# tungphambasement/DCNN

Measured on AMD Instinct MI355X. Metric: images/sec (whole node) ResNet-18 Tiny-ImageNet training at 1/2/4/8 MI355X, higher is better.
Workload: dtype bf16; 1 GPU; model=resnet18_tiny_imagenet, global_batch=256, per_gpu_batch=256, parallelism=dp1, optimizer=adam, hipgraph=True, engine=native (C++ host API)

## Files before the change

### dcnn_amd/csrc/host/dcnn/nn.hpp

```cpp
#pragma once
#include <functional>
#include <map>
#include <memory>
#include <string>
#include <vector>

#include "json.hpp"
#include "ops.hpp"
#include "tensor.hpp"

namespace dcnn {

struct ParamArena;
struct Param {
  std::string name;
  std::vector<int64_t> shape;
  Layout layout = Layout::NCHW;
  Tensor value, grad, shadow;
  Tensor m, v;
  std::shared_ptr<ParamArena> arena;
};

struct ParamArena {
  Tensor value, grad, m, v, shadow;
// ... 119 lines not shown
  std::string type() const override { return "grouped_conv2d"; }
  json::Value parameters_config() const override;
  bool backward_residual(const Tensor& dy, const Tensor& residual, Tensor& dx) override;
};

class Dense : public Layer {
 public:
  Dense(int in_features, int out_features, bool bias = true, std::string name = "dense");
  std::string type() const override { return "dense"; }
  json::Value parameters_config() const override;
  std::vector<int64_t> output_shape(const std::vector<int64_t>& in) const override;
  void build(const std::vector<int64_t>& in, Device dev, uint64_t seed) override;
  Tensor forward(const Tensor& x, bool training) override;
  Tensor backward(const Tensor& dy) override;
  double flops(const std::vector<int64_t>& in) const override { return 6.0 * in[0] * in_ * out_; }

 private:
  int in_, out_;
  bool bias_;
};

class BatchNorm : public Layer {
 public:
  explicit BatchNorm(int num_features, float eps = 1e-5f, float momentum = 0.1f, bool affine = true,
                     std::string name = "batchnorm");
  std::string type() const override { return "batchnorm"; }
  json::Value parameters_config() const override;
  std::vector<int64_t> output_shape(const std::vector<int64_t>& in) const override { return in; }
  double flops(const std::vector<int64_t>& in) const override {
    return 15.0 * (double)in[0] * (double)in[1] * (double)in[2] * (double)in[3];
  }
  void build(const std::vector<int64_t>& in, Device dev, uint64_t seed) override;
  Tensor forward(const Tensor& x, bool training) override;
  Tensor backward(const Tensor& dy) override;
// ... 89 lines not shown
};

class Pool2D : public Layer {
 public:
  Pool2D(bool max, int kh, int kw, int sh, int sw, int ph, int pw, std::string name);
  std::string type() const override { return max_ ? "maxpool2d" : "avgpool2d"; }
  json::Value parameters_config() const override;
  std::vector<int64_t> output_shape(const std::vector<int64_t>& in) const override;
  Tensor forward(const Tensor& x, bool training) override;
  Tensor backward(const Tensor& dy) override;
  bool is_max() const { return max_; }
  PoolShape shape_for(const std::vector<int64_t>& in) const;
  void set_fused_producer(class BatchNorm* bn) { bn_ = bn; }
  uint8_t* accept_prepooled(const Tensor& ypool, const std::vector<int64_t>& in);
  void clear_prepooled() { mbc().flag = false; }

 private:
  class BatchNorm* bn_ = nullptr;
  bool max_;
  int kh_, kw_, sh_, sw_, ph_, pw_;
};

class Flatten : public Layer {
 public:
  explicit Flatten(std::string name = "flatten") : Layer(std::move(name)) {}
  std::string type() const override { return "flatten"; }
  json::Value parameters_config() const override { return json::Value::object(); }
  std::vector<int64_t> output_shape(const std::vector<int64_t>& in) const override;
  Tensor forward(const Tensor& x, bool training) override;
  Tensor backward(const Tensor& dy) override;
};

class ResidualBlock : public Layer {
 public:
  ResidualBlock(std::vector<std::unique_ptr<Layer>> main, std::vector<std::unique_ptr<Layer>> shortcut,
                std::string activation = "relu", std::string name = "residual_block");
  std::string type() const override { return "residual_block"; }
  json::Value parameters_config() const override;
  std::vector<int64_t> output_shape(const std::vector<int64_t>& in) const override;
  double flops(const std::vector<int64_t>& in) const override;
  void build(const std::vector<int64_t>& in, Device dev, uint64_t seed) override;
  Tensor forward(const Tensor& x, bool training) override;
  Tensor backward(const Tensor& dy) override;
  void sync_shadow() override;
  void collect_params(std::vector<Param*>& out) override;
// ... 198 lines not shown
```

### dcnn_amd/csrc/host/dcnn/ops.hpp

```cpp
#pragma once
#include <cstdint>

namespace dcnn {

struct ConvShape {
  int N, C, H, W, Co, KH, KW, SH, SW, PH, PW, OH, OW;
};
struct PoolShape {
  int N, C, H, W, OH, OW, KH, KW, SH, SW, PH, PW;
};
enum ActKind { ACT_RELU = 0, ACT_LEAKY_RELU = 1, ACT_ELU = 2, ACT_SIGMOID = 3, ACT_TANH = 4, ACT_LINEAR = 5 };

namespace cpu_ops {
void conv_fwd(const float* x, const float* w, const float* b, float* y, const ConvShape& s);
void conv_bwd(const float* x, const float* w, const float* dy, float* dx, float* dw, float* db, const ConvShape& s);
void dwconv_fwd(const float* x, const float* w, const float* b, float* y, const ConvShape& s);
void dwconv_bwd(const float* x, const float* w, const float* dy, float* dx, float* dw, float* db, const ConvShape& s);
void gconv_fwd(const float* x, const float* w, const float* b, float* y, const ConvShape& s, int groups);
void gconv_bwd(const float* x, const float* w, const float* dy, float* dx, float* dw, float* db, const ConvShape& s,
               int groups);
void dense_fwd(const float* x, const float* w, const float* b, float* y, long N, long In, long Out);
void dense_bwd(const float* x, const float* w, const float* dy, float* dx, float* dw, float* db, long N, long In,
               long Out);
void bn_fwd(const float* x, float* y, long N, long C, long HW, const float* g, const float* b, float eps, bool train,
// ... 63 lines not shown
struct StemBn {
  const void* x;
  const float* mean;
  const float* istd;
  const float* gamma;
  float* dgamma;
  float* dbeta;
  const float* slab;
  int rows;
  bool train;
};
void stem_wgrad_bn(const void* dy, const float* x, float* gw, float* gb, const ConvShape& s, const StemBn& bn);
void dense_fwd(const void* x, const void* w, const float* bias, void* y, int N, int In, int Out);
void dense_dgrad(const void* dy, const void* w, void* dx, int N, int In, int Out);
void dense_wgrad(const void* dy, const void* x, float* gw, float* gb, int N, int In, int Out);
void bn_fwd(const void* x, void* y, long R, int C, const float* g, const float* b, float eps, bool train,
            float* rmean, float* rvar, float momentum, float* smean, float* sistd, bool relu = false,
            const void* residual = nullptr);
void bn_fwd_slab(const void* x, void* y, long R, int C, const float* slab, int rows, const float* g, const float* b,
                 float eps, float* rmean, float* rvar, float momentum, float* smean, float* sistd, bool relu,
                 const void* residual = nullptr);
void bn_bwd_slab(const void* dy, const void* x, void* dx, long R, int C, const float* mean, const float* istd,
                 const float* g, float* dg, float* db, bool train, const float* slab, int rows);
void bn_bwd(const void* dy, const void* x, void* dx, long R, int C, const float* mean, const float* istd,
            const float* g, float* dg, float* db, bool train, const void* yout = nullptr, void* dy_out = nullptr);
struct SecondaryStats {
  SecondaryStats();
  ~SecondaryStats();
};
struct BnRaw {
// ... 67 lines not shown
```

### dcnn_amd/csrc/host/nn.cpp

```cpp
#include "dcnn/nn.hpp"

#include "../kernels/fusion_plan.h"

#include <algorithm>
#include <chrono>
#include <cmath>
#include <cstdio>
#include <cstdlib>
#include <filesystem>
#include <fstream>
#include <iostream>
#include <sstream>
#include <stdexcept>

namespace dcnn {

namespace {
struct Rng {
  uint64_t s;
  explicit Rng(uint64_t seed) : s(seed * 0x9e3779b97f4a7c15ull + 0x632be59bd9b4e019ull) {}
  uint64_t next() {
    uint64_t z = (s += 0x9e3779b97f4a7c15ull);
    z = (z ^ (z >> 30)) * 0xbf58476d1ce4e5b9ull;
    z = (z ^ (z >> 27)) * 0x94d049bb133111ebull;
// ... 364 lines not shown
  if (in[1] * in[2] * in[3] != in_)
    throw std::runtime_error(name_ + ": " + std::to_string(in[1] * in[2] * in[3]) + " input features, expected " +
                             std::to_string(in_));
  return {in[0], out_, 1, 1};
}

void Dense::build(const std::vector<int64_t>& in, Device dev, uint64_t seed) {
  (void)in;
  dev_ = dev;
  params_.clear();
  const float bound = 1.f / std::sqrt((float)in_);
  add_param("weights", {out_, in_, 1, 1}, Layout::NCHW, uniform_init((size_t)out_ * in_, bound, seed));
  if (bias_) add_param("bias", {out_, 1, 1, 1}, Layout::NCHW, uniform_init((size_t)out_, bound, seed + 1));
}

Tensor Dense::forward(const Tensor& x, bool training) {
  (void)training;
  Tensor& x_ = mbc().a;
  check_act(x, dev_, "dense");
  const int N = (int)x.dim(0);
  output_shape(x.shape());
  Tensor y = act_empty({N, out_, 1, 1}, dev_);
  const float* b = bias_ ? params_[1].value.ptr<float>() : nullptr;
  if (dev_.is_gpu())
    gpu_ops::dense_fwd(x.data(), params_[0].shadow.data(), b, y.data(), N, in_, out_);
  else
    cpu_ops::dense_fwd(x.ptr<float>(), params_[0].value.ptr<float>(), b, y.ptr<float>(), N, in_, out_);
  x_ = x;
  return y;
}

Tensor Dense::backward(const Tensor& dy) {
  const Tensor& x_ = mbc().a;
  const int N = (int)x_.dim(0);
  float* gb = bias_ ? params_[1].grad.ptr<float>() : nullptr;
  if (dev_.is_gpu()) {
    gpu_ops::dense_wgrad(dy.data(), x_.data(), params_[0].grad.ptr<float>(), gb, N, in_, out_);
    if (!input_grad_) return Tensor();
    Tensor dx = act_empty(x_.shape(), dev_);
    gpu_ops::dense_dgrad(dy.data(), params_[0].shadow.data(), dx.data(), N, in_, out_);
    return dx;
  }
  Tensor dx = act_empty(x_.shape(), dev_);
  {
    cpu_ops::dense_bwd(x_.ptr<float>(), params_[0].value.ptr<float>(), dy.ptr<float>(), dx.ptr<float>(),
                       params_[0].grad.ptr<float>(), gb, N, in_, out_);
  }
  return dx;
}

// ... 274 lines not shown

json::Value Activation::parameters_config() const {
  json::Value p = json::Value::object();
  p["activation"] = kind_;
  return p;
}

static float act_alpha(int code) { return code == ACT_ELU ? 1.0f : 0.01f; }

bool Activation::is_relu() const { return code_ == ACT_RELU; }

static int fuse_kind(const Layer* l) {
  if (dynamic_cast<const Conv2D*>(l)) return FK_CONV;
  if (dynamic_cast<const BatchNorm*>(l)) return FK_BN;
  if (auto* a = dynamic_cast<const Activation*>(l)) return a->is_relu() ? FK_RELU : FK_ACT;
  if (auto* p = dynamic_cast<const Pool2D*>(l)) return p->is_max() ? FK_MAXPOOL : FK_OTHER;
  return FK_OTHER;
}

static std::vector<int> fuse_kinds(const std::vector<std::unique_ptr<Layer>>& seq) {
  std::vector<int> k;
  for (const auto& l : seq) k.push_back(fuse_kind(l.get()));
  return k;
}

void fuse_bn_relu(std::vector<std::unique_ptr<Layer>>& seq, bool on) {
  const std::vector<int> f = plan_sequence_fusions(fuse_kinds(seq));
  for (size_t i = 0; i < seq.size(); ++i) {
    Layer* l = seq[i].get();
    if (auto* conv = dynamic_cast<Conv2D*>(l)) {
      conv->set_stats_consumer(on && (f[i] & FF_EMIT_BN_STATS) ? static_cast<BatchNorm*>(seq[i + 1].get()) : nullptr);
      BatchNorm* prod = nullptr;
      if (on && (f[i] & FF_BNB_CONSUMER))
        prod = static_cast<BatchNorm*>(seq[fuse_kind(seq[i - 1].get()) == FK_BN ? i - 1 : i - 2].get());
      conv->set_bnb_producer(prod);
    } else if (auto* bn = dynamic_cast<BatchNorm*>(l)) {
      bn->set_fused_relu(on && (f[i] & FF_FUSE_RELU));
      Pool2D* pool = on && (f[i] & FF_FUSE_POOL) ? static_cast<Pool2D*>(seq[i + 2].get()) : nullptr;
      bn->set_fused_pool(pool);
      if (pool) pool->set_fused_producer(bn);
    } else if (auto* act = dynamic_cast<Activation*>(l)) {
      act->set_passthrough(on && (f[i] & FF_PASSTHROUGH));
    } else if (auto* pool = dynamic_cast<Pool2D*>(l)) {
      if (!on || i < 2 || !(f[i - 2] & FF_FUSE_POOL)) pool->set_fused_producer(nullptr);
    }
  }
}

Tensor Activation::forward(const Tensor& x, bool training) {
  (void)training;
  if (passthrough_ && dev_.is_gpu()) return x;
  Tensor& x_ = mbc().a;
  Tensor& y_ = mbc().b;
  check_act(x, dev_, "activation");
  Tensor y = act_empty(x.shape(), dev_);
  const long N = x.dim(0), C = x.dim(1), HW = x.dim(2) * x.dim(3);
  if (code_ == ACT_SOFTMAX) {
    if (dev_.is_gpu())
      gpu_ops::softmax_fwd(x.data(), y.data(), N * HW, (int)C);
// ... 390 lines not shown
  mc.b = ypool;
  mc.shape = in;
  mc.flag = true;
  return mc.a.ptr<uint8_t>();
}

Tensor Pool2D::forward(const Tensor& x, bool training) {
  (void)training;
  if (bn_ != nullptr && mbc().flag && mbc().b.defined() && mbc().b.data() == x.data())
    return x;
  mbc().flag = false;
  Tensor& idx_ = mbc().a;
  std::vector<int64_t>& in_shape_ = mbc().shape;
  check_act(x, dev_, "pool2d");
  const PoolShape p = shape_for(x.shape());
  Tensor y = act_empty({p.N, p.C, p.OH, p.OW}, dev_);
  in_shape_ = x.shape();
  if (max_) {
    const int64_t n = (int64_t)p.N * p.C * p.OH * p.OW;
    if (dev_.is_gpu()) {
      idx_.ensure({n}, DType::U8, dev_);
      gpu_ops::maxpool_fwd(x.data(), y.data(), idx_.ptr<uint8_t>(), p);
    } else {
      idx_.ensure({n}, DType::I32, dev_);
      cpu_ops::maxpool_fwd(x.ptr<float>(), y.ptr<float>(), idx_.ptr<int32_t>(), p);
    }
  } else if (dev_.is_gpu()) {
    gpu_ops::avgpool_fwd(x.data(), y.data(), p);
  } else {
    cpu_ops::avgpool_fwd(x.ptr<float>(), y.ptr<float>(), p);
  }
  return y;
}

Tensor Pool2D::backward(const Tensor& dy) {
  const Tensor& idx_ = mbc().a;
  const std::vector<int64_t>& in_shape_ = mbc().shape;
  const PoolShape p = shape_for(in_shape_);
  Tensor dx = act_empty(in_shape_, dev_);
  if (mbc().flag && bn_ != nullptr) {
    const gpu_ops::BnbOperands ops = bn_->bnb_operands(mb_);
    int rows = 0;
    const float* slab = gpu_ops::maxpool_bwd_bnb(dy.data(), idx_.ptr<uint8_t>(), mbc().b.data(), ops.x, ops.mean,
                                                 ops.istd, dx.data(), p, &rows);
    bn_->offer_bwd_stats(dx.data(), slab, rows);
    return dx;
  }
  if (max_) {
    if (dev_.is_gpu())
      gpu_ops::maxpool_bwd(dy.data(), idx_.ptr<uint8_t>(), dx.data(), p);
// ... 14 lines not shown
Tensor Flatten::forward(const Tensor& x, bool training) {
  (void)training;
  std::vector<int64_t>& in_shape_ = mbc().shape;
  check_act(x, dev_, "flatten");
  in_shape_ = x.shape();
  const auto os = output_shape(x.shape());
  const int64_t HW = x.dim(2) * x.dim(3);
  if (!dev_.is_gpu()) return x.view(os);
  if (HW == 1) return x.view(os, Layout::NHWC);
  Tensor y = act_empty(os, dev_);
  gpu_ops::nhwc_to_nchw(x.data(), y.data(), (int)x.dim(0), (int)HW, (int)x.dim(1));
  return y;
}

Tensor Flatten::backward(const Tensor& dy) {
  const std::vector<int64_t>& in_shape_ = mbc().shape;
  const int64_t HW = in_shape_[2] * in_shape_[3];
  if (!dev_.is_gpu()) return dy.view(in_shape_);
  if (HW == 1) return dy.view(in_shape_, Layout::NHWC);
  Tensor dx = act_empty(in_shape_, dev_);
  gpu_ops::nchw_to_nhwc_bf16(dy.data(), dx.data(), (int)in_shape_[0], (int)HW, (int)in_shape_[1]);
  return dx;
}

std::unique_ptr<Layer> create_layer(const json::Value& rec) {
  const std::string type = rec.get_string("type", "");
  const std::string name = rec.get_string("name", type);
  static const json::Value empty = json::Value::object();
  const json::Value& p = rec.has("parameters") ? rec.at("parameters") : empty;
  auto I = [&](const char* k, int64_t d) { return (int)p.get_int(k, d); };
// ... 711 lines not shown
```

### dcnn_amd/csrc/host/ops_gpu.hip

```cpp
#include <hip/hip_runtime.h>

#include <algorithm>
#include <cmath>
#include <cstdio>
#include <cstdlib>
#include <cstring>
#include <map>
#include <mutex>
#include <stdexcept>
#include <string>
#include <unordered_map>
#include <vector>

#include "../kernels/api.h"
#include "dcnn/ops.hpp"
#include "dcnn/tensor.hpp"

#define HOST_HIP_CHECK(x)                                                                    \
  do {                                                                                       \
    hipError_t e_ = (x);                                                                     \
    if (e_ != hipSuccess) throw std::runtime_error(std::string(#x) + ": " + hipGetErrorString(e_)); \
  } while (0)

namespace dcnn {
// ... 758 lines not shown
  conv_weight_transpose(kBF16, w, wt, Out, 1, In, cur());
  NtArgs a{static_cast<const bf16*>(dy), wt, dx, N, In, Out, Out, Out, In, kPlain, 0, 0, 0, 0, 1, 1, 1, 1, 1, 1, 0, 0,
           nullptr, nullptr, nullptr, 0, 0};
  gemm_nt(a, cur());
}

void dense_wgrad(const void* dy, const void* x, float* gw, float* gb, int N, int In, int Out) {
  const int splits = gemm_tn_splits(Out, In, N);
  wgrad_split(splits, (long)Out * In, Out, gw, gb, [&](float* slab, float* bslab) {
    TnArgs a{static_cast<const bf16*>(dy), static_cast<const bf16*>(x), slab, bslab, Out, In, N, kPlain, 0, 0, 0, 0,
             1, 1, 1, 1, 1, 1, 0, 0, In, 0};
    gemm_tn(a, splits, cur());
  });
}

static std::pair<const float*, int> reduce_stats(int mode, const float* slab, int rows, int C) {
  const int parts = bn_stat_parts(rows);
  float* sums = static_cast<float*>(scratch(STAT_SUMS, (size_t)2 * C * 4));
  float* part = parts > 1 ? static_cast<float*>(scratch(STAT_PART, (size_t)parts * 3 * C * 4)) : nullptr;
  bn_stat_reduce(mode, slab, rows, C, sums, part, nullptr, cur());
  return {parts > 1 ? part : sums, parts};
}

void bn_fwd(const void* x, void* y, long R, int C, const float* g, const float* b, float eps, bool train,
            float* rmean, float* rvar, float momentum, float* smean, float* sistd, bool relu, const void* residual) {
  if (!train) {
    bn_apply(kBF16, x, y, R, C, nullptr, 1, (float)R, g, b, eps, residual, relu ? 1 : 0, smean, sistd, rmean, rvar,
             momentum, 1, cur());
    return;
  }
// ... 228 lines not shown
```

### dcnn_amd/csrc/kernels/api.h

```cpp
#pragma once
#include <hip/hip_runtime.h>
#include <stdint.h>

#include "fusion_plan.h"
typedef __bf16 bf16;

namespace dcnn {
struct BnbArgs {
  const bf16* y; const bf16* x; const float* mean; const float* istd;
  const float* gamma; const float* beta; int mask_x;
};
struct NtArgs {
  const bf16* A; const bf16* B; void* C;
  int M, N, K; int lda, ldb, ldc; int mode;
  int nb, sh, sw, cs, gh, gw; int kh, kw, strh, strw, padh, padw;
  const float* bias; const bf16* residual; float* stats; int out_f32; int relu;
};
struct TnArgs {
  const bf16* dY; const bf16* X; float* slab; float* bias_slab;
  int M, N, P; int mode; int nb, sh, sw, cs, gh, gw; int kh, kw, strh, strw, padh, padw; int ldx; int k_per_split;
};
struct G2Args {
  const bf16* A; const bf16* B; bf16* C;
  unsigned a_bytes, b_bytes;
// ... 107 lines not shown
void transpose_batched(const float* in, float* out, int batch, int rows, int cols, hipStream_t s);
void transpose_batched16(const void* in, void* out, int batch, int rows, int cols, hipStream_t s);
void rows_copy(int kind, const void* src, int lds, void* dst, int ldd, long rows, int cols, hipStream_t s);
void nchw_cnhw(const float* in, float* out, int N, int C, int HW, int to_cnhw, hipStream_t s);
void pad_crop(const float* in, float* out, int NC, int H, int W, int OH, int OW, int top, int left, float value,
              hipStream_t s);
void gemm_g2f(const G2Args& a, hipStream_t s);
int gemm_g2f_stat_rows(int M, int N);
void gemm_t2f(T2Args a, int splits, hipStream_t s);
int gemm_t2f_splits(int M, int N, int P);
void set_f32_mode(int mode);
int get_f32_mode();
void conv_weight_transpose_f32(const float* w, float* wt, int Co, int T_, int Ci, hipStream_t s);
void gemm_tn(TnArgs a, int splits, hipStream_t s);
int gemm_tn_splits(int M, int N, int P);
struct ConvRouteGeom {
  int N, C, H, W, Co, KH, KW, SH, SW, PH, PW, OH, OW, g1s_mode;
};
enum ConvRoute : int { ROUTE_GENERIC = 0, ROUTE_GEMM_G2 = 1, ROUTE_HALO = 2, ROUTE_G1S = 3, ROUTE_HALO_S2 = 4 };
int conv_fwd_route(ConvRouteGeom g);
int conv_dgrad_route(ConvRouteGeom g);
int conv_wgrad_route(ConvRouteGeom g);
void splitk_reduce(const float* slab, float* out, long n, int splits, int accumulate, hipStream_t s);
void splitk_reduce2(const float* slab, float* out, long n, const float* bslab, float* bout, long nb, int splits,
                    int accumulate, hipStream_t s);

constexpr int kMaxRed = 48;
struct RedEnt { const float* slab; float* out; long n; int splits, unit0, chunks, groups, vec, wpc; };
struct MultiRed { int count; RedEnt e[kMaxRed]; };
void multi_splitk_reduce(MultiRed t, hipStream_t s);
// ... 28 lines not shown
                     const float* gamma, const float* beta, float eps, float* save_mean, float* save_istd,
                     float* run_mean, float* run_var, float momentum, hipStream_t s);
void gn_fwd(int dtype, const void* x, void* y, int N, int HW, int C, int G, const float* gamma, const float* beta,
            float eps, float* save_mean, float* save_istd, hipStream_t s);
void gn_bwd(int dtype, const void* dy, const void* x, void* dx, int N, int HW, int C, int G, const float* gamma,
            const float* mean, const float* istd, float* dgamma, float* dbeta, float* aff, hipStream_t s);

void maxpool_fwd(int dt, const void* x, void* y, uint8_t* idx, PoolGeom g, hipStream_t s);
void maxpool_bwd(int dt, const void* dy, const uint8_t* idx, void* dx, PoolGeom g, hipStream_t s);
bool maxpool_bwd_bnb_supported(PoolGeom g);
int maxpool_bwd_bnb_rows(PoolGeom g);
void maxpool_bwd_bnb(const bf16* dy, const uint8_t* idx, const bf16* ypool, const bf16* x, const float* mean,
                     const float* istd, bf16* dx, PoolGeom g, float* slab, float* zero_sums, hipStream_t s);
void avgpool_fwd(int dt, const void* x, void* y, PoolGeom g, hipStream_t s);
void avgpool_bwd(int dt, const void* dy, void* dx, PoolGeom g, hipStream_t s);
void act_fwd(int dt, const void* x, void* y, long n, int type, float a, hipStream_t s);
void act_bwd(int dt, const void* x, const void* dy, void* dx, long n, int type, float a, hipStream_t s);
void softmax_rows(int dt, const void* x, void* y, long rows, int C, hipStream_t s);
void softmax_rows_bwd(int dt, const void* y, const void* dy, void* dx, long rows, int C, hipStream_t s);
void dropout(int dt, const void* x, void* y, long n, float p, uint64_t seed, const uint64_t* ctr, hipStream_t s);
void counter_bump(uint64_t* ctr, uint64_t* slot, hipStream_t s);
void nchw_to_nhwc(int dt, const float* x, void* y, int N, int C, int HW, hipStream_t s);
void nchw_to_nhwc_pad(int dt, const float* x, void* y, int N, int C, int Cp, int HW, hipStream_t s);
void conv_weight_transpose(int src_dt, const void* w, bf16* wt, int Co, int T_, int Ci, hipStream_t s);
void cast_f32_bf16(const float* x, bf16* y, long n, hipStream_t s);
struct StemArgs {
  const float* x; const void* w; int w_bf16; long ws[4];
  const float* bias; bf16* y; float* slab; float* zero_ptr; int zero_n;
  const bf16* dy; float* bias_slab; long gs[4]; long n_slab;
  int halo_bytes; int N, Ci, H, W, Co, TH;
// ... 59 lines not shown
```

### dcnn_amd/csrc/kernels/bindings.cpp

```cpp
#include <tuple>
#include <pybind11/pybind11.h>
#include <pybind11/stl.h>
#include <algorithm>
#include <array>
#include <vector>
#include <hip/hip_runtime.h>
#include <stdint.h>

namespace py = pybind11;
#include "api.h"


using namespace dcnn;
void bind_runtime(py::module_& m);
void bind_rccl(py::module_& m);
template <typename T>
static inline T P(uintptr_t x) { return reinterpret_cast<T>(x); }
static inline hipStream_t S(uintptr_t x) { return reinterpret_cast<hipStream_t>(x); }

using Ptr4 = std::array<uintptr_t, 4>;
static BnbArgs bnb_of(const Ptr4& b) {
  return BnbArgs{P<const bf16*>(b[0]), P<const bf16*>(b[1]), P<const float*>(b[2]), P<const float*>(b[3])};
}

// ... 186 lines not shown
    std::vector<std::array<int, 6>> ph;
    for (const DgradPhase& c : p.phases) ph.push_back({c.ry, c.rx, c.GH, c.GW, c.t0, c.nt});
    return std::make_pair(ph, p.taps);
  });
  m.attr("ROUTE_GENERIC") = (int)ROUTE_GENERIC;
  m.attr("ROUTE_GEMM_G2") = (int)ROUTE_GEMM_G2;
  m.attr("ROUTE_HALO") = (int)ROUTE_HALO;
  m.attr("ROUTE_G1S") = (int)ROUTE_G1S;
  m.attr("ROUTE_HALO_S2") = (int)ROUTE_HALO_S2;
  m.def("plan_sequence_fusions", &plan_sequence_fusions);
  m.def("plan_residual_fusions", &plan_residual_fusions);
  for (auto [name, v] : {std::pair<const char*, int>{"FK_OTHER", FK_OTHER}, {"FK_CONV", FK_CONV}, {"FK_BN", FK_BN},
                         {"FK_RELU", FK_RELU}, {"FK_ACT", FK_ACT}, {"FK_MAXPOOL", FK_MAXPOOL},
                         {"FF_EMIT_BN_STATS", FF_EMIT_BN_STATS}, {"FF_FUSE_RELU", FF_FUSE_RELU},
                         {"FF_PASSTHROUGH", FF_PASSTHROUGH}, {"FF_FUSE_POOL", FF_FUSE_POOL},
                         {"FF_BNB_CONSUMER", FF_BNB_CONSUMER}, {"RF_FUSED_TAIL", RF_FUSED_TAIL},
                         {"RF_DUAL_SHORTCUT", RF_DUAL_SHORTCUT}})
    m.attr(name) = v;
  m.def("g1s_rows", &g1s_rows);
  m.def("g1s_enable", &g1s_enable);
  m.def("g1s_set_waves_per_simd", &g1s_set_waves_per_simd);
  m.def("g1s_gen_rows", &g1s_gen_rows);
  m.def("g1s_gen", [](uintptr_t X, uintptr_t Wt, uintptr_t Y, int NB, int GH, int GW, int N, int Kc, int ldw,
                      std::vector<std::array<int, 3>> taps, int H, int W, int OHo, int OWo, int OS, int ORY, int ORX,
                      uintptr_t residual, uintptr_t stats, uintptr_t zero_ptr, int zero_n, Ptr4 bnb,
                      int mode, uintptr_t stream) {
    g1s_gen(P<const bf16*>(X), P<const bf16*>(Wt), P<bf16*>(Y), NB, GH, GW, N, Kc, ldw, taps, H, W, OHo, OWo, OS, ORY,
            ORX, P<const bf16*>(residual), P<float*>(stats), P<float*>(zero_ptr), zero_n,
            bnb_of(bnb),
            mode, S(stream));
  });
// ... 182 lines not shown
  m.def("maxpool_bwd_bnb", [geom](uintptr_t dy, uintptr_t idx, uintptr_t ypool, uintptr_t x, uintptr_t mean,
                                  uintptr_t istd, uintptr_t dx, int N, int H, int W, int C, int OH, int OW, int ph,
                                  int pw, int sh, int sw, int padh, int padw, uintptr_t slab, uintptr_t zero_sums,
                                  uintptr_t st) {
    maxpool_bwd_bnb(P<const bf16*>(dy), P<const uint8_t*>(idx), P<const bf16*>(ypool), P<const bf16*>(x),
                    P<const float*>(mean), P<const float*>(istd), P<bf16*>(dx),
                    geom(N, H, W, C, OH, OW, ph, pw, sh, sw, padh, padw), P<float*>(slab), P<float*>(zero_sums), S(st));
  });
  m.def("avgpool_fwd", [geom](int dt, uintptr_t x, uintptr_t y, int N, int H, int W, int C, int OH, int OW, int ph,
                              int pw, int sh, int sw, int padh, int padw, uintptr_t st) {
    avgpool_fwd(dt, P<const void*>(x), P<void*>(y), geom(N, H, W, C, OH, OW, ph, pw, sh, sw, padh, padw), S(st));
  });
  m.def("avgpool_bwd", [geom](int dt, uintptr_t dy, uintptr_t dx, int N, int H, int W, int C, int OH, int OW, int ph,
                              int pw, int sh, int sw, int padh, int padw, uintptr_t st) {
    avgpool_bwd(dt, P<const void*>(dy), P<void*>(dx), geom(N, H, W, C, OH, OW, ph, pw, sh, sw, padh, padw), S(st));
  });
  m.def("act_fwd", [](int dt, uintptr_t x, uintptr_t y, long n, int type, float a, uintptr_t st) {
    act_fwd(dt, P<const void*>(x), P<void*>(y), n, type, a, S(st));
  });
  m.def("act_bwd", [](int dt, uintptr_t x, uintptr_t dy, uintptr_t dx, long n, int type, float a, uintptr_t st) {
    act_bwd(dt, P<const void*>(x), P<const void*>(dy), P<void*>(dx), n, type, a, S(st));
  });
  m.def("softmax_rows", [](int dt, uintptr_t x, uintptr_t y, long rows, int C, uintptr_t st) {
    softmax_rows(dt, P<const void*>(x), P<void*>(y), rows, C, S(st));
  });
  m.def("softmax_rows_bwd", [](int dt, uintptr_t y, uintptr_t dy, uintptr_t dx, long rows, int C, uintptr_t st) {
    softmax_rows_bwd(dt, P<const void*>(y), P<const void*>(dy), P<void*>(dx), rows, C, S(st));
  });
  m.def("dropout", [](int dt, uintptr_t x, uintptr_t y, long n, float p, uint64_t seed, uintptr_t ctr, uintptr_t st) {
    dropout(dt, P<const void*>(x), P<void*>(y), n, p, seed, P<const uint64_t*>(ctr), S(st));
// ... 128 lines not shown
```

### dcnn_amd/csrc/kernels/fusion_plan.cpp

```cpp
#include "fusion_plan.h"

namespace dcnn {

std::vector<int> plan_sequence_fusions(const std::vector<int>& kinds) {
  const size_t n = kinds.size();
  std::vector<int> f(n, 0);
  auto is = [&](size_t i, int k) { return i < n && kinds[i] == k; };
  for (size_t i = 0; i + 1 < n; ++i) {
    if (is(i, FK_CONV) && is(i + 1, FK_BN)) f[i] |= FF_EMIT_BN_STATS;
    if (is(i, FK_BN) && is(i + 1, FK_RELU)) {
      f[i] |= FF_FUSE_RELU;
      f[i + 1] |= FF_PASSTHROUGH;
    }
  }
  for (size_t i = 0; i + 2 < n; ++i)
    if (is(i, FK_BN) && is(i + 1, FK_RELU) && is(i + 2, FK_MAXPOOL)) f[i] |= FF_FUSE_POOL;
  for (size_t j = 1; j < n; ++j) {
    if (!is(j, FK_CONV)) continue;
    if (is(j - 1, FK_BN) || (j >= 2 && is(j - 1, FK_RELU) && is(j - 2, FK_BN))) f[j] |= FF_BNB_CONSUMER;
  }
  return f;
}

int plan_residual_fusions(const std::vector<int>& main_kinds, const std::vector<int>& short_kinds, bool act_ok) {
  const bool tail = act_ok && main_kinds.size() >= 2 && main_kinds.back() == FK_BN;
  if (!tail) return 0;
  const bool dual = !short_kinds.empty() && short_kinds.back() == FK_BN;
  return RF_FUSED_TAIL | (dual ? RF_DUAL_SHORTCUT : 0);
}

}
```

### dcnn_amd/csrc/kernels/fusion_plan.h

```cpp
#pragma once
#include <vector>

namespace dcnn {

enum FuseKind : int { FK_OTHER = 0, FK_CONV = 1, FK_BN = 2, FK_RELU = 3, FK_ACT = 4, FK_MAXPOOL = 5 };
enum FuseFlag : int {
  FF_EMIT_BN_STATS = 1,
  FF_FUSE_RELU = 2,
  FF_PASSTHROUGH = 4,
  FF_FUSE_POOL = 8,
  FF_BNB_CONSUMER = 16,
};
std::vector<int> plan_sequence_fusions(const std::vector<int>& kinds);
enum ResidualFlag : int { RF_FUSED_TAIL = 1, RF_DUAL_SHORTCUT = 2 };
int plan_residual_fusions(const std::vector<int>& main_kinds, const std::vector<int>& short_kinds, bool act_ok);

}
```

### dcnn_amd/csrc/kernels/gemm_conv.hip

```cpp
#include <algorithm>

#include "common.h"
#include "api.h"

namespace dcnn {

enum GatherMode { kPlain = 0, kConvFwd = 1, kConvDgrad = 2 };



__device__ __forceinline__ int xcd_remap(int bid, int nwg) {
  const int xcd = bid & 7, q = nwg >> 3, r = nwg & 7;
  const int base = xcd < r ? xcd * (q + 1) : r * (q + 1) + (xcd - r) * q;
  return base + (bid >> 3);
}

template <int BM, int BN, int BK, bool VEC>
struct NtTile {
  static constexpr int CPR = BK / 8;
  static constexpr int RPB = 256 / (BK * 2);
  static constexpr int A_CH = BM * CPR / 256;
  static constexpr int B_CH = BN * CPR / 256;
  static constexpr int TM = BM / 32, TN = BN / 32;
  static constexpr int LDS_BYTES = 2 * (BM + BN) * BK * 2;
// ... 625 lines not shown

int gemm_tn_splits(int M, int N, int P) {
  const int bm = M >= 128 ? 128 : 64, bn = N >= 128 ? 128 : 64;
  const long tiles = (long)((M + bm - 1) / bm) * ((N + bn - 1) / bn);
  long splits = (512 + tiles - 1) / tiles;
  const long min_k = tiles < 32 ? 64 : 64 * 4;
  const long max_by_k = P / min_k > 0 ? P / min_k : 1;
  if (splits > max_by_k) splits = max_by_k;
  const long max_by_mem = (64l << 20) / (4l * M * N) > 0 ? (64l << 20) / (4l * M * N) : 1;
  if (splits > max_by_mem) splits = max_by_mem;
  if (splits < 1) splits = 1;
  if (splits > 128) splits = 128;
  return (int)splits;
}

void gemm_tn(TnArgs a, int splits, hipStream_t s) {
  const bool conv = a.mode == kConvFwd;
  const int bm = a.M >= 128 ? 128 : 64;
  int bn = a.N >= 128 ? 128 : 64;
  if (conv) while (bn > 32 && a.cs % bn != 0) bn >>= 1;
  const bool v = a.M % 8 == 0 && (conv ? a.cs % bn == 0 : (a.N % 8 == 0 && a.ldx % 8 == 0));
  if (!v) bn = a.N >= 128 ? 128 : 64;
  const int per = (a.P + splits - 1) / splits;
  a.k_per_split = ((per + 63) / 64) * 64;
#define DCNN_TN(BM, BN, V) if (bm == BM && bn == BN && v == V) return launch_tn<BM, BN, 64, V>(a, splits, s)
  DCNN_TN(128, 128, true);
  DCNN_TN(128, 64, true);
  DCNN_TN(128, 32, true);
  DCNN_TN(64, 128, true);
  DCNN_TN(64, 64, true);
  DCNN_TN(64, 32, true);
  DCNN_TN(128, 128, false);
  DCNN_TN(128, 64, false);
  DCNN_TN(64, 128, false);
  DCNN_TN(64, 64, false);
#undef DCNN_TN
  throw std::runtime_error("gemm_tn: no kernel variant");
}

// ... 16 lines not shown
```

Before: 89810 images/sec.

## Fuse global avgpool, flatten and dense classifier head into single kernels

Adds a fused head path: the final whole-map average pool and the dense layer run in one forward kernel that writes both pooled features and logits. A single backward kernel computes the pool input gradient (dense dgrad broadcast over the spatial map) and the split weight gradients. Fusion planning tags an avgpool-flatten-dense tail, and the pool and flatten layers pass through when the fused path is active. This removes separate pool, dense GEMM and pool-backward launches and their intermediate traffic, at the cost of a specialised kernel with shape restrictions and extra cache bookkeeping between the layers.

```diff
diff --git a/dcnn_amd/csrc/host/dcnn/nn.hpp b/dcnn_amd/csrc/host/dcnn/nn.hpp
--- a/dcnn_amd/csrc/host/dcnn/nn.hpp
+++ b/dcnn_amd/csrc/host/dcnn/nn.hpp
@@ -157,10 +157,14 @@
   Tensor forward(const Tensor& x, bool training) override;
   Tensor backward(const Tensor& dy) override;
   double flops(const std::vector<int64_t>& in) const override { return 6.0 * in[0] * in_ * out_; }
+  void set_head_pool(class Pool2D* p) { head_pool_ = p; }
+  bool run_head(const Tensor& x, const PoolShape& p, Tensor& pooled);
+  bool is_head_dx(const Tensor& dy, bool take);
 
  private:
   int in_, out_;
   bool bias_;
+  class Pool2D* head_pool_ = nullptr;
 };
 
 class BatchNorm : public Layer {
@@ -280,9 +284,11 @@
   void set_fused_producer(class BatchNorm* bn) { bn_ = bn; }
   uint8_t* accept_prepooled(const Tensor& ypool, const std::vector<int64_t>& in);
   void clear_prepooled() { mbc().flag = false; }
+  void set_head_dense(class Dense* d) { head_ = d; }
 
  private:
   class BatchNorm* bn_ = nullptr;
+  class Dense* head_ = nullptr;
   bool max_;
   int kh_, kw_, sh_, sw_, ph_, pw_;
 };
@@ -295,6 +301,10 @@
   std::vector<int64_t> output_shape(const std::vector<int64_t>& in) const override;
   Tensor forward(const Tensor& x, bool training) override;
   Tensor backward(const Tensor& dy) override;
+  void set_head_dense(class Dense* d) { head_ = d; }
+
+ private:
+  class Dense* head_ = nullptr;
 };
 
 class ResidualBlock : public Layer {
diff --git a/dcnn_amd/csrc/host/dcnn/ops.hpp b/dcnn_amd/csrc/host/dcnn/ops.hpp
--- a/dcnn_amd/csrc/host/dcnn/ops.hpp
+++ b/dcnn_amd/csrc/host/dcnn/ops.hpp
@@ -101,6 +101,10 @@
 void dense_fwd(const void* x, const void* w, const float* bias, void* y, int N, int In, int Out);
 void dense_dgrad(const void* dy, const void* w, void* dx, int N, int In, int Out);
 void dense_wgrad(const void* dy, const void* x, float* gw, float* gb, int N, int In, int Out);
+bool head_supported(const PoolShape& p, int Out);
+void head_fwd(const void* x, const void* w, const float* bias, void* pooled, void* y, const PoolShape& p, int Out);
+void head_bwd(const void* dy, const void* w, const void* pooled, void* dx, float* gw, float* gb, const PoolShape& p,
+              int Out);
 void bn_fwd(const void* x, void* y, long R, int C, const float* g, const float* b, float eps, bool train,
             float* rmean, float* rvar, float momentum, float* smean, float* sistd, bool relu = false,
             const void* residual = nullptr);
diff --git a/dcnn_amd/csrc/host/nn.cpp b/dcnn_amd/csrc/host/nn.cpp
--- a/dcnn_amd/csrc/host/nn.cpp
+++ b/dcnn_amd/csrc/host/nn.cpp
@@ -402,8 +402,51 @@
   if (bias_) add_param("bias", {out_, 1, 1, 1}, Layout::NCHW, uniform_init((size_t)out_, bound, seed + 1));
 }
 
+static bool head_fuse_enabled() {
+  static const bool on = [] {
+    const char* v = std::getenv("DCNN_HEAD_FUSE");
+    return !(v && std::string(v) == "0");
+  }();
+  return on;
+}
+
+bool Dense::run_head(const Tensor& x, const PoolShape& p, Tensor& pooled) {
+  MbCache& mc = mbc();
+  mc.flag = false;
+  if (!dev_.is_gpu() || !head_fuse_enabled() || p.C != in_ || !gpu_ops::head_supported(p, out_)) return false;
+  pooled = act_empty({p.N, p.C, 1, 1}, dev_);
+  Tensor y = act_empty({p.N, out_, 1, 1}, dev_);
+  const float* b = bias_ ? params_[1].value.ptr<float>() : nullptr;
+  gpu_ops::head_fwd(x.data(), params_[0].shadow.data(), b, pooled.data(), y.data(), p, out_);
+  mc.a = pooled;
+  mc.b = y;
+  mc.shape = x.shape();
+  mc.flag = true;
+  return true;
+}
+
+bool Dense::is_head_dx(const Tensor& dy, bool take) {
+  MbCache& mc = mbc();
+  if (head_pool_ == nullptr || mc.u == 0) return false;
+  const bool same = mc.c.defined() ? dy.defined() && dy.data() == mc.c.data() : !dy.defined();
+  if (same && take) {
+    mc.c = Tensor();
+    mc.u = 0;
+  }
+  return same;
+}
+
 Tensor Dense::forward(const Tensor& x, bool training) {
   (void)training;
+  mbc().c = Tensor();
+  mbc().u = 0;
+  if (mbc().flag && mbc().b.defined() && x.data() == mbc().a.data()) {
+    Tensor y = mbc().b;
+    mbc().b = Tensor();
+    return y;
+  }
+  mbc().flag = false;
+  mbc().b = Tensor();
   Tensor& x_ = mbc().a;
   check_act(x, dev_, "dense");
   const int N = (int)x.dim(0);
@@ -422,6 +465,15 @@
   const Tensor& x_ = mbc().a;
   const int N = (int)x_.dim(0);
   float* gb = bias_ ? params_[1].grad.ptr<float>() : nullptr;
+  if (head_pool_ != nullptr && mbc().flag) {
+    const PoolShape p = head_pool_->shape_for(mbc().shape);
+    Tensor dx = input_grad_ ? act_empty(mbc().shape, dev_) : Tensor();
+    gpu_ops::head_bwd(dy.data(), params_[0].shadow.data(), x_.data(), input_grad_ ? dx.data() : nullptr,
+                      params_[0].grad.ptr<float>(), gb, p, out_);
+    mbc().c = dx;
+    mbc().u = 1;
+    return dx;
+  }
   if (dev_.is_gpu()) {
     gpu_ops::dense_wgrad(dy.data(), x_.data(), params_[0].grad.ptr<float>(), gb, N, in_, out_);
     if (!input_grad_) return Tensor();
@@ -726,7 +778,9 @@
   if (dynamic_cast<const Conv2D*>(l)) return FK_CONV;
   if (dynamic_cast<const BatchNorm*>(l)) return FK_BN;
   if (auto* a = dynamic_cast<const Activation*>(l)) return a->is_relu() ? FK_RELU : FK_ACT;
-  if (auto* p = dynamic_cast<const Pool2D*>(l)) return p->is_max() ? FK_MAXPOOL : FK_OTHER;
+  if (auto* p = dynamic_cast<const Pool2D*>(l)) return p->is_max() ? FK_MAXPOOL : FK_AVGPOOL;
+  if (dynamic_cast<const Flatten*>(l)) return FK_FLATTEN;
+  if (dynamic_cast<const Dense*>(l)) return FK_DENSE;
   return FK_OTHER;
 }
 
@@ -755,6 +809,11 @@
       act->set_passthrough(on && (f[i] & FF_PASSTHROUGH));
     } else if (auto* pool = dynamic_cast<Pool2D*>(l)) {
       if (!on || i < 2 || !(f[i - 2] & FF_FUSE_POOL)) pool->set_fused_producer(nullptr);
+      pool->set_head_dense(on && (f[i] & FF_FUSE_HEAD) ? static_cast<Dense*>(seq[i + 2].get()) : nullptr);
+    } else if (auto* flat = dynamic_cast<Flatten*>(l)) {
+      flat->set_head_dense(on && i >= 1 && (f[i - 1] & FF_FUSE_HEAD) ? static_cast<Dense*>(seq[i + 1].get()) : nullptr);
+    } else if (auto* dense = dynamic_cast<Dense*>(l)) {
+      dense->set_head_pool(on && i >= 2 && (f[i - 2] & FF_FUSE_HEAD) ? static_cast<Pool2D*>(seq[i - 2].get()) : nullptr);
     }
   }
 }
@@ -1175,8 +1234,13 @@
   std::vector<int64_t>& in_shape_ = mbc().shape;
   check_act(x, dev_, "pool2d");
   const PoolShape p = shape_for(x.shape());
+  in_shape_ = x.shape();
+  if (head_ != nullptr && training && !max_) {
+    head_->set_micro_batch(mb_);
+    Tensor pooled;
+    if (head_->run_head(x, p, pooled)) return pooled;
+  }
   Tensor y = act_empty({p.N, p.C, p.OH, p.OW}, dev_);
-  in_shape_ = x.shape();
   if (max_) {
     const int64_t n = (int64_t)p.N * p.C * p.OH * p.OW;
     if (dev_.is_gpu()) {
@@ -1195,6 +1259,10 @@
 }
 
 Tensor Pool2D::backward(const Tensor& dy) {
+  if (head_ != nullptr) {
+    head_->set_micro_batch(mb_);
+    if (head_->is_head_dx(dy, true)) return dy;
+  }
   const Tensor& idx_ = mbc().a;
   const std::vector<int64_t>& in_shape_ = mbc().shape;
   const PoolShape p = shape_for(in_shape_);
@@ -1239,6 +1307,10 @@
 }
 
 Tensor Flatten::backward(const Tensor& dy) {
+  if (head_ != nullptr) {
+    head_->set_micro_batch(mb_);
+    if (head_->is_head_dx(dy, false)) return dy;
+  }
   const std::vector<int64_t>& in_shape_ = mbc().shape;
   const int64_t HW = in_shape_[2] * in_shape_[3];
   if (!dev_.is_gpu()) return dy.view(in_shape_);
diff --git a/dcnn_amd/csrc/host/ops_gpu.hip b/dcnn_amd/csrc/host/ops_gpu.hip
--- a/dcnn_amd/csrc/host/ops_gpu.hip
+++ b/dcnn_amd/csrc/host/ops_gpu.hip
@@ -796,6 +796,21 @@
   });
 }
 
+bool head_supported(const PoolShape& p, int Out) { return dcnn::head_supported(geom(p), Out); }
+
+void head_fwd(const void* x, const void* w, const float* bias, void* pooled, void* y, const PoolShape& p, int Out) {
+  dcnn::head_fwd(static_cast<const bf16*>(x), static_cast<const bf16*>(w), bias, static_cast<bf16*>(pooled),
+                 static_cast<bf16*>(y), geom(p), Out, cur());
+}
+
+void head_bwd(const void* dy, const void* w, const void* pooled, void* dx, float* gw, float* gb, const PoolShape& p,
+              int Out) {
+  wgrad_split(head_bwd_splits(p.N, p.C, Out), (long)Out * p.C, Out, gw, gb, [&](float* slab, float* bslab) {
+    dcnn::head_bwd(static_cast<const bf16*>(dy), static_cast<const bf16*>(w), static_cast<const bf16*>(pooled),
+                   static_cast<bf16*>(dx), slab, bslab, geom(p), Out, cur());
+  });
+}
+
 static std::pair<const float*, int> reduce_stats(int mode, const float* slab, int rows, int C) {
   const int parts = bn_stat_parts(rows);
   float* sums = static_cast<float*>(scratch(STAT_SUMS, (size_t)2 * C * 4));
diff --git a/dcnn_amd/csrc/kernels/api.h b/dcnn_amd/csrc/kernels/api.h
--- a/dcnn_amd/csrc/kernels/api.h
+++ b/dcnn_amd/csrc/kernels/api.h
@@ -145,6 +145,8 @@
 void conv_weight_transpose_f32(const float* w, float* wt, int Co, int T_, int Ci, hipStream_t s);
 void gemm_tn(TnArgs a, int splits, hipStream_t s);
 int gemm_tn_splits(int M, int N, int P);
+int gemm_tn_k_per_split(int P, int splits);
+int gemm_tn_bias_rows(int M);
 struct ConvRouteGeom {
   int N, C, H, W, Co, KH, KW, SH, SW, PH, PW, OH, OW, g1s_mode;
 };
@@ -203,6 +205,12 @@
                      const float* istd, bf16* dx, PoolGeom g, float* slab, float* zero_sums, hipStream_t s);
 void avgpool_fwd(int dt, const void* x, void* y, PoolGeom g, hipStream_t s);
 void avgpool_bwd(int dt, const void* dy, void* dx, PoolGeom g, hipStream_t s);
+bool head_supported(PoolGeom g, int Out);
+void head_fwd(const bf16* x, const bf16* w, const float* bias, bf16* pooled, bf16* logits, PoolGeom g, int Out,
+              hipStream_t s);
+int head_bwd_splits(int N, int In, int Out);
+void head_bwd(const bf16* dlogits, const bf16* w, const bf16* pooled, bf16* dx, float* slab, float* bias_slab,
+              PoolGeom g, int Out, hipStream_t s);
 void act_fwd(int dt, const void* x, void* y, long n, int type, float a, hipStream_t s);
 void act_bwd(int dt, const void* x, const void* dy, void* dx, long n, int type, float a, hipStream_t s);
 void softmax_rows(int dt, const void* x, void* y, long rows, int C, hipStream_t s);
diff --git a/dcnn_amd/csrc/kernels/bindings.cpp b/dcnn_amd/csrc/kernels/bindings.cpp
--- a/dcnn_amd/csrc/kernels/bindings.cpp
+++ b/dcnn_amd/csrc/kernels/bindings.cpp
@@ -224,7 +224,9 @@
                          {"FK_RELU", FK_RELU}, {"FK_ACT", FK_ACT}, {"FK_MAXPOOL", FK_MAXPOOL},
                          {"FF_EMIT_BN_STATS", FF_EMIT_BN_STATS}, {"FF_FUSE_RELU", FF_FUSE_RELU},
                          {"FF_PASSTHROUGH", FF_PASSTHROUGH}, {"FF_FUSE_POOL", FF_FUSE_POOL},
-                         {"FF_BNB_CONSUMER", FF_BNB_CONSUMER}, {"RF_FUSED_TAIL", RF_FUSED_TAIL},
+                         {"FF_BNB_CONSUMER", FF_BNB_CONSUMER}, {"FK_AVGPOOL", FK_AVGPOOL},
+                         {"FK_FLATTEN", FK_FLATTEN}, {"FK_DENSE", FK_DENSE}, {"FF_FUSE_HEAD", FF_FUSE_HEAD},
+                         {"RF_FUSED_TAIL", RF_FUSED_TAIL},
                          {"RF_DUAL_SHORTCUT", RF_DUAL_SHORTCUT}})
     m.attr(name) = v;
   m.def("g1s_rows", &g1s_rows);
@@ -437,6 +439,23 @@
   m.def("avgpool_bwd", [geom](int dt, uintptr_t dy, uintptr_t dx, int N, int H, int W, int C, int OH, int OW, int ph,
                               int pw, int sh, int sw, int padh, int padw, uintptr_t st) {
     avgpool_bwd(dt, P<const void*>(dy), P<void*>(dx), geom(N, H, W, C, OH, OW, ph, pw, sh, sw, padh, padw), S(st));
+  });
+  m.def("head_supported", [geom](int N, int H, int W, int C, int OH, int OW, int ph, int pw, int sh, int sw, int padh,
+                                 int padw, int Out) {
+    return head_supported(geom(N, H, W, C, OH, OW, ph, pw, sh, sw, padh, padw), Out);
+  });
+  m.def("head_fwd", [geom](uintptr_t x, uintptr_t w, uintptr_t bias, uintptr_t pooled, uintptr_t logits, int N, int H,
+                           int W, int C, int OH, int OW, int ph, int pw, int sh, int sw, int padh, int padw, int Out,
+                           uintptr_t st) {
+    head_fwd(P<const bf16*>(x), P<const bf16*>(w), P<const float*>(bias), P<bf16*>(pooled), P<bf16*>(logits),
+             geom(N, H, W, C, OH, OW, ph, pw, sh, sw, padh, padw), Out, S(st));
+  });
+  m.def("head_bwd_splits", &head_bwd_splits);
+  m.def("head_bwd", [geom](uintptr_t dlogits, uintptr_t w, uintptr_t pooled, uintptr_t dx, uintptr_t slab,
+                           uintptr_t bias_slab, int N, int H, int W, int C, int OH, int OW, int ph, int pw, int sh,
+                           int sw, int padh, int padw, int Out, uintptr_t st) {
+    head_bwd(P<const bf16*>(dlogits), P<const bf16*>(w), P<const bf16*>(pooled), P<bf16*>(dx), P<float*>(slab),
+             P<float*>(bias_slab), geom(N, H, W, C, OH, OW, ph, pw, sh, sw, padh, padw), Out, S(st));
   });
   m.def("act_fwd", [](int dt, uintptr_t x, uintptr_t y, long n, int type, float a, uintptr_t st) {
     act_fwd(dt, P<const void*>(x), P<void*>(y), n, type, a, S(st));
diff --git a/dcnn_amd/csrc/kernels/fusion_plan.cpp b/dcnn_amd/csrc/kernels/fusion_plan.cpp
--- a/dcnn_amd/csrc/kernels/fusion_plan.cpp
+++ b/dcnn_amd/csrc/kernels/fusion_plan.cpp
@@ -19,6 +19,7 @@
     if (!is(j, FK_CONV)) continue;
     if (is(j - 1, FK_BN) || (j >= 2 && is(j - 1, FK_RELU) && is(j - 2, FK_BN))) f[j] |= FF_BNB_CONSUMER;
   }
+  if (n >= 3 && is(n - 3, FK_AVGPOOL) && is(n - 2, FK_FLATTEN) && is(n - 1, FK_DENSE)) f[n - 3] |= FF_FUSE_HEAD;
   return f;
 }
 
diff --git a/dcnn_amd/csrc/kernels/fusion_plan.h b/dcnn_amd/csrc/kernels/fusion_plan.h
--- a/dcnn_amd/csrc/kernels/fusion_plan.h
+++ b/dcnn_amd/csrc/kernels/fusion_plan.h
@@ -3,13 +3,17 @@
 
 namespace dcnn {
 
-enum FuseKind : int { FK_OTHER = 0, FK_CONV = 1, FK_BN = 2, FK_RELU = 3, FK_ACT = 4, FK_MAXPOOL = 5 };
+enum FuseKind : int {
+  FK_OTHER = 0, FK_CONV = 1, FK_BN = 2, FK_RELU = 3, FK_ACT = 4, FK_MAXPOOL = 5, FK_AVGPOOL = 6, FK_FLATTEN = 7,
+  FK_DENSE = 8
+};
 enum FuseFlag : int {
   FF_EMIT_BN_STATS = 1,
   FF_FUSE_RELU = 2,
   FF_PASSTHROUGH = 4,
   FF_FUSE_POOL = 8,
   FF_BNB_CONSUMER = 16,
+  FF_FUSE_HEAD = 32,
 };
 std::vector<int> plan_sequence_fusions(const std::vector<int>& kinds);
 enum ResidualFlag : int { RF_FUSED_TAIL = 1, RF_DUAL_SHORTCUT = 2 };
diff --git a/dcnn_amd/csrc/kernels/gemm_conv.hip b/dcnn_amd/csrc/kernels/gemm_conv.hip
--- a/dcnn_amd/csrc/kernels/gemm_conv.hip
+++ b/dcnn_amd/csrc/kernels/gemm_conv.hip
@@ -663,6 +663,9 @@
   return (int)splits;
 }
 
+int gemm_tn_k_per_split(int P, int splits) { return ((P + splits - 1) / splits + 63) / 64 * 64; }
+int gemm_tn_bias_rows(int M) { return 256 / (M >= 128 ? 128 : 64); }
+
 void gemm_tn(TnArgs a, int splits, hipStream_t s) {
   const bool conv = a.mode == kConvFwd;
   const int bm = a.M >= 128 ? 128 : 64;
@@ -670,8 +673,7 @@
   if (conv) while (bn > 32 && a.cs % bn != 0) bn >>= 1;
   const bool v = a.M % 8 == 0 && (conv ? a.cs % bn == 0 : (a.N % 8 == 0 && a.ldx % 8 == 0));
   if (!v) bn = a.N >= 128 ? 128 : 64;
-  const int per = (a.P + splits - 1) / splits;
-  a.k_per_split = ((per + 63) / 64) * 64;
+  a.k_per_split = gemm_tn_k_per_split(a.P, splits);
 #define DCNN_TN(BM, BN, V) if (bm == BM && bn == BN && v == V) return launch_tn<BM, BN, 64, V>(a, splits, s)
   DCNN_TN(128, 128, true);
   DCNN_TN(128, 64, true);
diff --git a/dcnn_amd/csrc/kernels/head.hip b/dcnn_amd/csrc/kernels/head.hip
--- /dev/null
+++ b/dcnn_amd/csrc/kernels/head.hip
@@ -0,0 +1,293 @@
+#include <algorithm>
+
+#include "api.h"
+#include "common.h"
+
+namespace dcnn {
+namespace {
+
+constexpr int kImgs = 16;
+constexpr int kFwdThreads = 512;
+constexpr int kFwdCls = 128;
+constexpr int kBwdThreads = 256;
+constexpr int kMaxIn = 2048;
+constexpr int kKC = 256;
+constexpr int kLdD = kKC + 8;
+constexpr int kLdW = 64 + 8;
+
+__device__ __forceinline__ f32x4 mfma16(bf16x8 a, bf16x8 b, f32x4 c) {
+  return __builtin_amdgcn_mfma_f32_16x16x32_bf16(a, b, c, 0, 0, 0);
+}
+__device__ __forceinline__ bf16x8 ld8(const bf16* p) { return *reinterpret_cast<const bf16x8*>(p); }
+
+__device__ __forceinline__ int swz(int r, int c) { return c ^ (r & 7); }
+
+__device__ __forceinline__ int wt_at(int i, int k) { return i * kLdD + (i >> 3) * 8 + k; }
+
+constexpr int kSmemData = (kImgs * kLdD + 64 * kLdD + 64 + kImgs * 64) * 2;
+constexpr int kSmemWeight = 2 * 64 * kLdW * 2;
+constexpr int kSmemBwd = kSmemData > kSmemWeight ? kSmemData : kSmemWeight;
+
+}
+
+__global__ __launch_bounds__(kFwdThreads) void head_fwd_kernel(const bf16* __restrict__ x, const bf16* __restrict__ w,
+                                                               const float* __restrict__ bias,
+                                                               bf16* __restrict__ pooled, bf16* __restrict__ logits,
+                                                               int N, int HW, int In, int Out, int ipb) {
+  extern __shared__ __attribute__((aligned(16))) unsigned char head_smem[];
+  bf16* tile = reinterpret_cast<bf16*>(head_smem);
+  const int n0 = blockIdx.x * ipb, nend = min(N, n0 + ipb);
+  const int chunks = In >> 3;
+  const int wave = threadIdx.x >> 6, lane = threadIdx.x & 63;
+  const int r = lane & 15, g = lane >> 4;
+  const int c0 = blockIdx.y * kFwdCls + wave * 16;
+  const bool wave_on = c0 < Out;
+  const int cls = c0 + r;
+  const bool cok = cls < Out;
+  const bf16* wr = w + (long)(cok ? cls : 0) * In + g * 8;
+  const int k64 = In >> 6;
+  bf16x8 b[16];
+  auto load_w = [&](int k0) {
+#pragma unroll
+    for (int u = 0; u < 8; ++u) {
+      const int kq = min(k0 + u, k64 - 1);
+      b[2 * u] = ld8(wr + kq * 64);
+      b[2 * u + 1] = ld8(wr + kq * 64 + 32);
+    }
+  };
+  if (wave_on) load_w(0);
+
+  for (int it = threadIdx.x; it < kImgs * chunks; it += kFwdThreads) {
+    const int pr = it / chunks, c = it - pr * chunks;
+    const int n = n0 + pr;
+    float s[8];
+#pragma unroll
+    for (int e = 0; e < 8; ++e) s[e] = 0.f;
+    if (n < nend) {
+      const uint4* px = reinterpret_cast<const uint4*>(x + (long)n * HW * In) + c;
+      for (int p0 = 0; p0 < HW; p0 += 8) {
+        uint4 u[8];
+#pragma unroll
+        for (int q = 0; q < 8; ++q) u[q] = p0 + q < HW ? px[(long)(p0 + q) * chunks] : make_uint4(0, 0, 0, 0);
+#pragma unroll
+        for (int q = 0; q < 8; ++q) {
+          float f[8];
+          unpack8(u[q], f);
+#pragma unroll
+          for (int e = 0; e < 8; ++e) s[e] += f[e];
+        }
+      }
+#pragma unroll
+      for (int e = 0; e < 8; ++e) s[e] = s[e] / (float)HW;
+    }
+    const uint4 o = pack8(s);
+    *reinterpret_cast<uint4*>(tile + pr * In + swz(pr, c) * 8) = o;
+    if (blockIdx.y == 0 && n < nend) *reinterpret_cast<uint4*>(pooled + (long)n * In + c * 8) = o;
+  }
+  __syncthreads();
+  if (!wave_on) return;
+
+  const bf16* ar = tile + r * In;
+  f32x4 acc = {0.f, 0.f, 0.f, 0.f};
+  for (int k0 = 0; k0 < k64; k0 += 8) {
+    if (k0 > 0) load_w(k0);
+#pragma unroll
+    for (int u = 0; u < 8; ++u) {
+      if (k0 + u < k64) {
+        acc = mfma16(ld8(ar + swz(r, (k0 + u) * 8 + g) * 8), b[2 * u], acc);
+        acc = mfma16(ld8(ar + swz(r, (k0 + u) * 8 + 4 + g) * 8), b[2 * u + 1], acc);
+      }
+    }
+  }
+  if (!cok) return;
+  const float bv = bias ? bias[cls] : 0.f;
+#pragma unroll
+  for (int j = 0; j < 4; ++j) {
+    const int n = n0 + g * 4 + j;
+    if (n < nend) logits[(long)n * Out + cls] = (bf16)(acc[j] + bv);
+  }
+}
+
+__global__ __launch_bounds__(kBwdThreads) void head_bwd_kernel(const bf16* __restrict__ dl, const bf16* __restrict__ w,
+                                                               const bf16* __restrict__ pooled, bf16* __restrict__ dx,
+                                                               float* __restrict__ slab, float* __restrict__ bslab,
+                                                               int N, int HW, int In, int Out, int n_data, int per,
+                                                               int brows) {
+  __shared__ __attribute__((aligned(16))) unsigned char smem[kSmemBwd];
+  const int tid = threadIdx.x, wave = tid >> 6, lane = tid & 63;
+  const int r = lane & 15, g = lane >> 4;
+  const int tiles_i = In >> 6;
+  const bf16 bz = (bf16)0.f;
+
+  if ((int)blockIdx.x < n_data) {
+    bf16* sdl = reinterpret_cast<bf16*>(smem);
+    bf16* swt = sdl + kImgs * kLdD;
+    bf16* sout = swt + 64 * kLdD + 64;
+    const int ib = blockIdx.x / tiles_i, cb = blockIdx.x - ib * tiles_i;
+    const int n0 = ib * kImgs, i0 = cb * 64;
+    f32x4 acc = {0.f, 0.f, 0.f, 0.f};
+    for (int o0 = 0; o0 < Out; o0 += kKC) {
+      const int kc = min(kKC, Out - o0);
+      const int kp = (kc + 31) & ~31;
+      if (o0 > 0) __syncthreads();
+      uint4 wv[kKC / 32];
+      bf16 dv[kKC / 16];
+      const int c8 = tid & 7, dr = tid >> 4;
+#pragma unroll
+      for (int it = 0; it < kKC / 32; ++it) {
+        const int k = (tid >> 3) + 32 * it;
+        wv[it] = k < kc ? *reinterpret_cast<const uint4*>(w + (long)(o0 + k) * In + i0 + c8 * 8) : make_uint4(0, 0, 0, 0);
+      }
+#pragma unroll
+      for (int it = 0; it < kKC / 16; ++it) {
+        const int k = (tid & 15) + 16 * it;
+        dv[it] = (n0 + dr < N && k < kc) ? dl[(long)(n0 + dr) * Out + o0 + k] : bz;
+      }
+#pragma unroll
+      for (int it = 0; it < kKC / 32; ++it) {
+        const int k = (tid >> 3) + 32 * it;
+        const bf16* v = reinterpret_cast<const bf16*>(&wv[it]);
+        if (k < kp) {
+#pragma unroll
+          for (int j = 0; j < 8; ++j) swt[wt_at(c8 * 8 + j, k)] = v[j];
+        }
+      }
+#pragma unroll
+      for (int it = 0; it < kKC / 16; ++it) {
+        const int k = (tid & 15) + 16 * it;
+        if (k < kp) sdl[dr * kLdD + k] = dv[it];
+      }
+      __syncthreads();
+      for (int kb = 0; kb < kp / 32; ++kb)
+        acc = mfma16(ld8(sdl + r * kLdD + kb * 32 + g * 8), ld8(swt + wt_at(wave * 16 + r, kb * 32 + g * 8)), acc);
+    }
+    const float inv = 1.f / (float)HW;
+#pragma unroll
+    for (int j = 0; j < 4; ++j) {
+      const bf16 dp = (bf16)(acc[j] + 0.f);
+      sout[(g * 4 + j) * 64 + wave * 16 + r] = (bf16)((float)dp * inv);
+    }
+    __syncthreads();
+    const int total = kImgs * HW * 8;
+    for (int e = tid; e < total; e += kBwdThreads) {
+      const int c8 = e & 7, q = e >> 3;
+      const int rr = q / HW, p = q - rr * HW;
+      const int n = n0 + rr;
+      if (n < N)
+        *reinterpret_cast<uint4*>(dx + ((long)n * HW + p) * In + i0 + c8 * 8) =
+            *reinterpret_cast<const uint4*>(sout + rr * 64 + c8 * 8);
+    }
+    return;
+  }
+
+  bf16* sa = reinterpret_cast<bf16*>(smem);
+  bf16* sb = sa + 64 * kLdW;
+  const int wb = blockIdx.x - n_data;
+  const int tiles_o = (Out + 63) >> 6;
+  const int split = wb / (tiles_o * tiles_i), t = wb - split * tiles_o * tiles_i;
+  const int ob = t / tiles_i, cb = t - ob * tiles_i;
+  const int o0 = ob * 64, i0 = cb * 64;
+  const int nbeg = split * per, nend = min(N, nbeg + per);
+  f32x4 acc[4];
+#pragma unroll
+  for (int q = 0; q < 4; ++q) acc[q] = f32x4{0.f, 0.f, 0.f, 0.f};
+  float bpart[4] = {0.f, 0.f, 0.f, 0.f};
+  for (int c0 = nbeg; c0 < nend; c0 += 64) {
+    if (c0 > nbeg) __syncthreads();
+    uint4 pv[2];
+    bf16 dv[16];
+    const int c8 = tid & 7, o = tid & 63;
+#pragma unroll
+    for (int it = 0; it < 2; ++it) {
+      const int nn = (tid >> 3) + 32 * it;
+      pv[it] = c0 + nn < nend ? *reinterpret_cast<const uint4*>(pooled + (long)(c0 + nn) * In + i0 + c8 * 8)
+                              : make_uint4(0, 0, 0, 0);
+    }
+#pragma unroll
+    for (int it = 0; it < 16; ++it) {
+      const int nn = (tid >> 6) + 4 * it;
+      dv[it] = (c0 + nn < nend && o0 + o < Out) ? dl[(long)(c0 + nn) * Out + o0 + o] : bz;
+    }
+#pragma unroll
+    for (int it = 0; it < 2; ++it) {
+      const int nn = (tid >> 3) + 32 * it;
+      const bf16* v = reinterpret_cast<const bf16*>(&pv[it]);
+#pragma unroll
+      for (int j = 0; j < 8; ++j) sb[(c8 * 8 + j) * kLdW + nn] = v[j];
+    }
+#pragma unroll
+    for (int it = 0; it < 16; ++it) sa[o * kLdW + (tid >> 6) + 4 * it] = dv[it];
+    __syncthreads();
+    for (int kb = 0; kb < 2; ++kb) {
+      const bf16x8 a = ld8(sa + (wave * 16 + r) * kLdW + kb * 32 + g * 8);
+#pragma unroll
+      for (int q = 0; q < 4; ++q) acc[q] = mfma16(a, ld8(sb + (q * 16 + r) * kLdW + kb * 32 + g * 8), acc[q]);
+    }
+    if (bslab != nullptr && cb == 0 && tid < 64) {
+      if (brows == 2) {
+        for (int nn = 0; nn < 64; ++nn) bpart[nn & 1] += (float)sa[tid * kLdW + nn];
+      } else {
+        for (int nn = 0; nn < 64; ++nn) bpart[nn & 3] += (float)sa[tid * kLdW + nn];
+      }
+    }
+  }
+  float* out = slab + (long)split * Out * In;
+#pragma unroll
+  for (int j = 0; j < 4; ++j) {
+    const int o = o0 + wave * 16 + g * 4 + j;
+    if (o < Out) {
+#pragma unroll
+      for (int q = 0; q < 4; ++q) out[(long)o * In + i0 + q * 16 + r] = acc[q][j];
+    }
+  }
+  if (bslab != nullptr && cb == 0 && tid < 64 && o0 + tid < Out) {
+    float bsum = 0.f;
+    for (int k = 0; k < brows; ++k) bsum += bpart[k];
+    bslab[(long)split * Out + o0 + tid] = bsum;
+  }
+}
+
+namespace {
+
+void check_head(PoolGeom g, int Out) {
+  if (!head_supported(g, Out))
+    throw std::invalid_argument("head: needs a whole-map average pool without padding, In % 64 == 0, In <= 2048, "
+                                "N >= 1, Out >= 1");
+}
+
+int head_per(int N, int In, int Out) { return gemm_tn_k_per_split(N, gemm_tn_splits(Out, In, N)); }
+
+}
+
+bool head_supported(PoolGeom g, int Out) {
+  return g.N >= 1 && Out >= 1 && g.H >= 1 && g.W >= 1 && g.OH == 1 && g.OW == 1 && g.ph == g.H && g.pw == g.W &&
+         g.padh == 0 && g.padw == 0 && g.C >= 64 && g.C % 64 == 0 && g.C <= kMaxIn &&
+         (long)g.N * g.H * g.W * g.C < (1l << 31) && (long)Out * g.C < (1l << 31) && (long)g.N * Out < (1l << 31);
+}
+
+void head_fwd(const bf16* x, const bf16* w, const float* bias, bf16* pooled, bf16* logits, PoolGeom g, int Out,
+              hipStream_t s) {
+  check_head(g, Out);
+  int ipb = kImgs;
+  while (ipb > 2 && (g.N + ipb - 1) / ipb < 32) ipb /= 2;
+  const dim3 grid((g.N + ipb - 1) / ipb, (Out + kFwdCls - 1) / kFwdCls);
+  hipLaunchKernelGGL(head_fwd_kernel, grid, dim3(kFwdThreads), (size_t)kImgs * g.C * 2, s, x, w, bias, pooled, logits,
+                     g.N, g.H * g.W, g.C, Out, ipb);
+  DCNN_LAUNCH_CHECK();
+}
+
+int head_bwd_splits(int N, int In, int Out) { return gemm_tn_splits(Out, In, N); }
+
+void head_bwd(const bf16* dlogits, const bf16* w, const bf16* pooled, bf16* dx, float* slab, float* bias_slab,
+              PoolGeom g, int Out, hipStream_t s) {
+  check_head(g, Out);
+  const int tiles_i = g.C / 64;
+  const int n_data = dx != nullptr ? (g.N + kImgs - 1) / kImgs * tiles_i : 0;
+  const int n_weight = head_bwd_splits(g.N, g.C, Out) * ((Out + 63) / 64) * tiles_i;
+  hipLaunchKernelGGL(head_bwd_kernel, dim3(n_data + n_weight), dim3(kBwdThreads), 0, s, dlogits, w, pooled, dx, slab,
+                     bias_slab, g.N, g.H * g.W, g.C, Out, n_data, head_per(g.N, g.C, Out),
+                     gemm_tn_bias_rows(Out));
+  DCNN_LAUNCH_CHECK();
+}
+
+}
```

Measured after the change: 91130 images/sec (median of 6 runs). +1.5%, better.
